# EthanD11/RS-VIO

Measured on AMD Instinct MI355X. Metric: stereo frames/sec (tracker+BA) on 752×480 EuRoC stream; BA ms/iter at window=10, higher is better.
Workload: dtype f32 (tracker) / f64 (BA)

## Files before the change

rs-vio_amd/csrc/pyramid.hip:

```cpp
#include "pyramid.hpp"

namespace rsvio {

namespace {

constexpr int TW = 64;
constexpr int TH = 8;
constexpr int STRIP_COLS = 320;
constexpr size_t LDS_CAP = 64 << 10;

__device__ __forceinline__ float triangle_kernel(float x) {
    float ax = fabsf(x);
    return ax < 1.0f ? 1.0f - ax : 0.0f;
}

__global__ void make_taps_kernel(TapTable tab, int n_entries) {
    int e = blockIdx.x * blockDim.x + threadIdx.x;
    if (e >= n_entries) return;
    int in_len = tab.ent_in_len[e];
    int out_len = tab.ent_out_len[e];
    int o = tab.ent_out_idx[e];
    float ratio = (float)in_len / (float)out_len;
    float sratio = ratio < 1.0f ? 1.0f : ratio;
    float support = 1.0f * sratio;
    float inputc = ((float)o + 0.5f) * ratio;
    long long left = (long long)floorf(inputc - support);
    if (left < 0) left = 0;
    if (left > (long long)in_len - 1) left = in_len - 1;
    long long right = (long long)ceilf(inputc + support);
    if (right < left + 1) right = left + 1;
    if (right > (long long)in_len) right = in_len;
    inputc = inputc - 0.5f;
    int cnt = (int)(right - left);
    float* w = tab.weights + (size_t)e * tab.max_taps;
    float sum = 0.0f;
    for (int k = 0; k < cnt; ++k) {
        float wv = triangle_kernel(((float)(left + k) - inputc) / sratio);
        w[k] = wv;
        sum += wv;
    }
    for (int k = 0; k < cnt; ++k) w[k] = w[k] / sum;
    tab.left[e] = (int)left;
    tab.count[e] = cnt;
}

__global__ __launch_bounds__(256) void pyramid_kernel(PyrLaunch L, PyrIO io) {
    extern __shared__ uint32_t smem[];
    const int img = blockIdx.y;
    {
        const int fb = (int)blockIdx.x - (L.copy_blocks + L.tile_start[L.levels]);
        if (fb >= 0) {
            if (io.table != nullptr) {
                const PyrSlot d = io.table[img];
                if (d.fast_pt != nullptr && fb < io.fast_cells)
                    fast_cell(d.src, io.fg, fb, nullptr, nullptr, 0, d.fast_pt, d.fast_aff,
                              reinterpret_cast<uint8_t*>(smem));
            } else if (img == 0 && fb < io.fast_cells) {
                const uint8_t* s0 = io.psrc ? io.psrc : io.src[0];
                fast_cell(s0, io.fg, fb, nullptr, nullptr, 0, io.fast_pt, io.fast_aff,
                          reinterpret_cast<uint8_t*>(smem));
            }
            return;
        }
    }
    const uint8_t* __restrict__ src =
        io.table ? io.table[img].src : (io.psrc ? io.psrc + (size_t)img * L.w * L.h : io.src[img]);
    uint8_t* __restrict__ dst_base =
        io.table ? io.table[img].dst : (io.psrc ? io.pdst + (size_t)img * L.pyr_bytes : io.dst[img]);
    int b = blockIdx.x;
    const bool aligned = ((reinterpret_cast<uintptr_t>(src) | reinterpret_cast<uintptr_t>(dst_base)) & 15) == 0;
    if (b < L.copy_blocks) {
        const size_t tot = (size_t)L.w * L.h;
        if (!aligned) {
            for (size_t i = (size_t)b * blockDim.x + threadIdx.x; i < tot; i += (size_t)L.copy_blocks * blockDim.x)
                dst_base[i] = src[i];
            return;
        }
        const size_t n16 = tot / 16;
        const uint4* s4 = reinterpret_cast<const uint4*>(src);
        uint4* d4 = reinterpret_cast<uint4*>(dst_base);
        for (size_t i = (size_t)b * blockDim.x + threadIdx.x; i < n16; i += (size_t)L.copy_blocks * blockDim.x)
            d4[i] = s4[i];
        size_t tail0 = n16 * 16;
        if (b == 0)
            for (size_t i = tail0 + threadIdx.x; i < tot; i += blockDim.x) dst_base[i] = src[i];
        return;
    }
    b -= L.copy_blocks;
    int lev = 1;
    while (lev < L.levels - 1 && b >= L.tile_start[lev + 1]) ++lev;
    b -= L.tile_start[lev];
    const int nw = (int)level_w(L.w, lev), nh = (int)level_h(L.h, lev);
    const int tw = L.tile_w[lev], th = L.tile_h[lev];
    const int tiles_x = (nw + tw - 1) / tw;
    const int tx = b % tiles_x, ty = b / tiles_x;
    const int ox0 = tx * tw, ox1 = min(ox0 + tw, nw);
    const int oy0 = ty * th, oy1 = min(oy0 + th, nh);
    const int rows = oy1 - oy0, cols_out = ox1 - ox0;
    const int hx = L.hx_ent[lev], vy = L.vy_ent[lev];
    const TapTable& T = L.tab;
    const int xl = T.left[hx + ox0];
    const int xr = T.left[hx + ox1 - 1] + T.count[hx + ox1 - 1];
    const int yl = T.left[vy + oy0];
    const int yr = T.left[vy + oy1 - 1] + T.count[vy + oy1 - 1];
    const int ncols = xr - xl, nrows = yr - yl;
    const int xa = xl & ~3, xoff = xl - xa;
    const int pd = (xr - xa + 3) >> 2;
    const bool direct = (L.direct >> lev) & 1;
    uint8_t* strip = reinterpret_cast<uint8_t*>(smem);
    if (!direct) {
        if (aligned && (L.w & 3) == 0) {
            const uint32_t* s32 = reinterpret_cast<const uint32_t*>(src);
            const int wd = (int)(L.w >> 2);
            for (int idx = threadIdx.x; idx < nrows * pd; idx += blockDim.x) {
                const int r = idx / pd, d = idx - r * pd;
                smem[idx] = s32[(size_t)(yl + r) * wd + (xa >> 2) + d];
            }
        } else {
            for (int idx = threadIdx.x; idx < nrows * pd * 4; idx += blockDim.x) {
                const int r = idx / (pd * 4), c = idx - r * pd * 4;
                strip[idx] = (xa + c < (int)L.w) ? src[(size_t)(yl + r) * L.w + xa + c] : 0;
            }
        }
    }
    float* tmp = reinterpret_cast<float*>(smem + (direct ? 0 : nrows * pd));
    __syncthreads();
    for (int idx = threadIdx.x; idx < rows * ncols; idx += blockDim.x) {
        const int r = idx / ncols, c = idx - r * ncols;
        const int e = vy + oy0 + r;
        const int vl = T.left[e], vc = T.count[e];
        const float* __restrict__ vw = T.weights + (size_t)e * T.max_taps;
        float acc = 0.0f;
        if (!direct) {
            const uint8_t* col = strip + (vl - yl) * pd * 4 + xoff + c;
            for (int k = 0; k < vc; ++k) acc += (float)col[k * pd * 4] * vw[k];
        } else {
            const uint8_t* __restrict__ col = src + (size_t)vl * L.w + xl + c;
            for (int k = 0; k < vc; k += 8) {
                float px[8];
#pragma unroll
                for (int u = 0; u < 8; ++u) px[u] = (k + u < vc) ? (float)col[(size_t)(k + u) * L.w] : 0.0f;
#pragma unroll
                for (int u = 0; u < 8; ++u)
                    if (k + u < vc) acc += px[u] * vw[k + u];
            }
        }
        tmp[r * ncols + c] = acc;
    }
    __syncthreads();
    uint8_t* __restrict__ dst = dst_base + level_offset(L.w, L.h, lev);
    for (int idx = threadIdx.x; idx < rows * cols_out; idx += blockDim.x) {
        const int r = idx / cols_out, c = idx - r * cols_out;
        const int e = hx + ox0 + c;
        const int hl = T.left[e] - xl, hc = T.count[e];
        const float* __restrict__ hw = T.weights + (size_t)e * T.max_taps;
        const float* __restrict__ row = tmp + r * ncols + hl;
        float acc = 0.0f;
        for (int k = 0; k < hc; ++k) acc += row[k] * hw[k];
        float cl = acc < 0.0f ? 0.0f : (acc > 255.0f ? 255.0f : acc);
        dst[(size_t)(oy0 + r) * nw + ox0 + c] = (uint8_t)roundf(cl);
    }
}

}

void PyramidPlan::init(int w_, int h_, int levels_) {
    w = w_;
    h = h_;
    levels = levels_;
    if (levels < 1 || levels > kMaxLevels) throw std::invalid_argument("levels must be in [1, 8]");
    if (w < 16 || h < 16) throw std::invalid_argument("image too small");
    std::vector<int> in_len, out_len, out_idx;
    float max_ratio = 1.0f;
    memset(&launch, 0, sizeof(launch));
    for (int i = 1; i < levels; ++i) {
        int nw = (int)level_w(w, i), nh = (int)level_h(h, i);
        if (nw < 1 || nh < 1) throw std::invalid_argument("too many levels for image size");
        launch.hx_ent[i] = (int)in_len.size();
        for (int o = 0; o < nw; ++o) { in_len.push_back(w); out_len.push_back(nw); out_idx.push_back(o); }
        launch.vy_ent[i] = (int)in_len.size();
        for (int o = 0; o < nh; ++o) { in_len.push_back(h); out_len.push_back(nh); out_idx.push_back(o); }
        float rx = (float)w / nw, ry = (float)h / nh;
        max_ratio = std::max(max_ratio, std::max(rx, ry));
        launch.tile_h[i] = std::max(1, std::min(TH, (int)(16.0f / ry)));
        launch.tile_w[i] = std::max(1, std::min(TW, (int)std::floor((STRIP_COLS - 2.0f * rx - 4.0f) / rx)));
    }
    n_entries = (int)in_len.size();
    max_taps = (int)std::ceil(2.0f * max_ratio) + 4;
    int tiles = 0;
    for (int i = 1; i < levels; ++i) {
        launch.tile_start[i] = tiles;
        int nw = (int)level_w(w, i), nh = (int)level_h(h, i);
        tiles += ((nw + launch.tile_w[i] - 1) / launch.tile_w[i]) * ((nh + launch.tile_h[i] - 1) / launch.tile_h[i]);
    }
    launch.tile_start[levels] = tiles;
    launch.copy_blocks = std::max(1, (int)(((size_t)w * h / 16 + 255) / 256 / 4));
    total_blocks = launch.copy_blocks + tiles;
    launch.w = (uint32_t)w;
    launch.h = (uint32_t)h;
    launch.levels = levels;
    launch.pyr_bytes = level_offset(w, h, levels);
    if (n_entries > 0) {
        i_in.alloc(n_entries); i_out.alloc(n_entries); i_idx.alloc(n_entries);
        d_left.alloc(n_entries); d_count.alloc(n_entries);
        d_w.alloc((size_t)n_entries * max_taps);
        RSVIO_HIP(hipMemcpy(i_in.p, in_len.data(), sizeof(int) * n_entries, hipMemcpyHostToDevice));
        RSVIO_HIP(hipMemcpy(i_out.p, out_len.data(), sizeof(int) * n_entries, hipMemcpyHostToDevice));
        RSVIO_HIP(hipMemcpy(i_idx.p, out_idx.data(), sizeof(int) * n_entries, hipMemcpyHostToDevice));
        TapTable t;
        t.left = d_left.p; t.count = d_count.p; t.weights = d_w.p; t.max_taps = max_taps;
        t.ent_in_len = i_in.p; t.ent_out_len = i_out.p; t.ent_out_idx = i_idx.p;
        hipLaunchKernelGGL(make_taps_kernel, dim3((n_entries + 255) / 256), dim3(256), 0, 0, t, n_entries);
        RSVIO_HIP(hipGetLastError());
        RSVIO_HIP(hipDeviceSynchronize());
        launch.tab = t;
        std::vector<int> left(n_entries), count(n_entries);
        RSVIO_HIP(hipMemcpy(left.data(), d_left.p, sizeof(int) * n_entries, hipMemcpyDeviceToHost));
        RSVIO_HIP(hipMemcpy(count.data(), d_count.p, sizeof(int) * n_entries, hipMemcpyDeviceToHost));
        for (int i = 1; i < levels; ++i) {
            const int nw = (int)level_w(w, i), nh = (int)level_h(h, i);
            const int tw = launch.tile_w[i], th = launch.tile_h[i];
            size_t strip = 0, vert = 0;
            for (int ox0 = 0; ox0 < nw; ox0 += tw) {
                const int ox1 = std::min(ox0 + tw, nw);
                const int xl = left[launch.hx_ent[i] + ox0];
                const int xr = left[launch.hx_ent[i] + ox1 - 1] + count[launch.hx_ent[i] + ox1 - 1];
                const size_t pd = (size_t)(xr - (xl & ~3) + 3) / 4;
                for (int oy0 = 0; oy0 < nh; oy0 += th) {
                    const int oy1 = std::min(oy0 + th, nh);
                    const int yl = left[launch.vy_ent[i] + oy0];
                    const int yr = left[launch.vy_ent[i] + oy1 - 1] + count[launch.vy_ent[i] + oy1 - 1];
                    strip = std::max(strip, 4 * pd * (size_t)(yr - yl));
                    vert = std::max(vert, 4 * (size_t)(oy1 - oy0) * (size_t)(xr - xl));
                }
            }
            if (vert > LDS_CAP) throw std::invalid_argument("image too wide for the pyramid tile");
            if (strip + vert > LDS_CAP) launch.direct |= 1u << i;
            lds_bytes = std::max(lds_bytes, ((launch.direct >> i) & 1) ? vert : strip + vert);
        }
    }
}

void PyramidPlan::enqueue(const PyrIO& io, int n_img, hipStream_t s) const {
    if (n_img <= 0) return;
    if (n_img > (io.psrc || io.table ? 65535 : kMaxPyrIO)) throw std::invalid_argument("too many images per pyramid launch");
    const size_t lds = io.fast_cells > 0 ? std::max(lds_bytes, (size_t)io.fg.g * io.fg.g) : lds_bytes;
    hipLaunchKernelGGL(pyramid_kernel, dim3(total_blocks + std::max(io.fast_cells, 0), n_img), dim3(256), lds, s,
                       launch, io);
    RSVIO_HIP(hipGetLastError());
}

void PyramidPlan::enqueue(const uint8_t* d_imgs, int n_img, uint8_t* d_pyrs, hipStream_t s) const {
    for (int i0 = 0; i0 < n_img; i0 += 65535) {
        PyrIO io{};
        io.psrc = d_imgs + (size_t)i0 * w * h;
        io.pdst = d_pyrs + (size_t)i0 * pyr_bytes();
        enqueue(io, std::min(65535, n_img - i0), s);
    }
}

}
```

rs-vio_amd/csrc/pyramid.hpp:

```cpp
#pragma once
#include <algorithm>
#include <cmath>
#include <cstring>
#include <stdexcept>
#include <vector>

#include "common.hpp"
#include "fast.hpp"

namespace rsvio {

constexpr int kMaxLevels = 8;

struct TapTable {
    int* left = nullptr;
    int* count = nullptr;
    float* weights = nullptr;
    int max_taps = 0;
    const int* ent_in_len = nullptr;
    const int* ent_out_len = nullptr;
    const int* ent_out_idx = nullptr;
};

struct PyrLaunch {
    uint32_t w, h;
    int levels;
    size_t pyr_bytes;
    int copy_blocks;
    int tile_start[kMaxLevels + 1];
    int tile_w[kMaxLevels];
    int tile_h[kMaxLevels];
    uint32_t direct;
    int hx_ent[kMaxLevels];
    int vy_ent[kMaxLevels];
    TapTable tab;
};

constexpr int kMaxPyrIO = 8;
struct PyrSlot {
    const uint8_t* src;
    uint8_t* dst;
    int4* fast_pt;
    float* fast_aff;
};
struct PyrIO {
    const uint8_t* src[kMaxPyrIO];
    uint8_t* dst[kMaxPyrIO];
    const uint8_t* psrc;
    uint8_t* pdst;
    int fast_cells;
    GridGeom fg;
    int4* fast_pt;
    float* fast_aff;
    const PyrSlot* table;
};

struct PyramidPlan {
    int w = 0, h = 0, levels = 0;
    int n_entries = 0, max_taps = 0, total_blocks = 0;
    size_t lds_bytes = 0;
    PyrLaunch launch;
    DevBuf<int> i_in, i_out, i_idx, d_left, d_count;
    DevBuf<float> d_w;
    void init(int w, int h, int levels);
    size_t pyr_bytes() const { return level_offset(w, h, levels); }
    void enqueue(const uint8_t* d_imgs, int n_img, uint8_t* d_pyrs, hipStream_t s) const;
    void enqueue(const PyrIO& io, int n_img, hipStream_t s) const;
};

}
```

rs-vio_amd/csrc/tracker.hip:

```cpp
#include <cmath>
#include <cstring>
#include <mutex>
#include <stdexcept>
#include <string>
#include <vector>

#include "lk_track.hpp"
#include "pyramid.hpp"
#include "camera.hpp"
#include "fast.hpp"

namespace rsvio {

namespace {

thread_local std::string g_last_error;

__device__ int block_exclusive_scan(int v, int* sh, int* total) {
    const int tid = threadIdx.x, lane = tid & 63, wave = tid >> 6, nw = blockDim.x >> 6;
    int incl = v;
#pragma unroll
    for (int off = 1; off < 64; off <<= 1) {
        const int t = __shfl_up(incl, off, 64);
        if (lane >= off) incl += t;
// ... 1060 lines not shown
            float* out[2] = {seeds_l, seeds_r};
            const size_t cp[2] = {cap_l, cap_r};
            std::vector<uint8_t> f;
            for (int k = 0; k < 2; ++k) {
                const size_t n = (size_t)T.pred_n[slot][k];
                f.assign(n, 0);
                if (n) RSVIO_HIP(hipMemcpy(f.data(), T.pflag(slot, k), n, hipMemcpyDeviceToHost));
                for (size_t i = 0; i < n; ++i) (f[i] ? c.n_seeded : c.n_unseeded)[k] += 1;
                if (!out[k]) continue;
                const size_t m = std::min(n, cp[k]);
                if (m) RSVIO_HIP(hipMemcpy(out[k], T.pseed(slot, k), m * sizeof(float2), hipMemcpyDeviceToHost));
                truncated = truncated || m < n;
            }
        }
        if (counts) *counts = c;
        if (truncated) {
            rsvio::set_last_error("rsvio_tracker_prediction_report: more seeds than the output capacity (truncated)");
            return (int)RSVIO_ERR_CAPACITY;
        }
        return (int)RSVIO_OK;
    });
}

int rsvio_tracker_remove_ids(rsvio_tracker* t, const uint64_t* ids, size_t n) {
    if (!t || (!ids && n)) return RSVIO_ERR_INVALID_ARG;
    if (n == 0) return RSVIO_OK;
    return guarded([&] {
        auto& T = t->t;
        T.require_collected("rsvio_tracker_remove_ids");
        if (T.rm_ids.n < n) T.rm_ids.alloc(n);
        RSVIO_HIP(hipMemcpyAsync(T.rm_ids.p, ids, n * sizeof(uint64_t), hipMemcpyHostToDevice, T.stream));
        hipLaunchKernelGGL(rsvio::remove_ids_kernel, dim3(1), dim3(1024), 0, T.stream, T.rm_ids.p, (int)n, T.maff(0),
                           T.maff(1), T.mid(0), T.mid(1), T.tmp_aff.p, T.ids_tmp.p, T.counts.p, T.outp(T.rslot, 0),
                           T.outp(T.rslot, 1), T.undp(T.rslot, 0), T.undp(T.rslot, 1), T.tmp_und.p);
        RSVIO_HIP(hipGetLastError());
        RSVIO_HIP(hipMemcpyAsync(T.h_counts.p, T.counts.p, sizeof(int) * 2, hipMemcpyDeviceToHost, T.stream));
        RSVIO_HIP(hipStreamSynchronize(T.stream));
        T.host_count[0] = T.h_counts.p[0];
        T.host_count[1] = T.h_counts.p[1];
        T.coll_n[0] = std::min(T.host_count[0], T.cap);
        T.coll_n[1] = std::min(T.host_count[1], T.cap);
        if (T.cams.on) {
            const size_t nl = std::min(T.last_n[0], (size_t)T.host_count[0]);
            const size_t nr = std::min(T.last_n[1], (size_t)T.host_count[1]);
            if (nl) RSVIO_HIP(hipMemcpyAsync(T.hund(T.rslot, 0), T.undp(T.rslot, 0), nl * sizeof(float2), hipMemcpyDeviceToHost, T.stream));
            if (nr) RSVIO_HIP(hipMemcpyAsync(T.hund(T.rslot, 1), T.undp(T.rslot, 1), nr * sizeof(float2),
                                             hipMemcpyDeviceToHost, T.stream));
            RSVIO_HIP(hipStreamSynchronize(T.stream));
            T.last_n[0] = nl;
            T.last_n[1] = nr;
        }
        return (int)RSVIO_OK;
    });
}

size_t rsvio_pyramid_bytes(int32_t w, int32_t h, int32_t levels) {
    if (w <= 0 || h <= 0 || levels <= 0) return 0;
    return rsvio::level_offset((uint32_t)w, (uint32_t)h, levels);
}

int rsvio_track_ctx_create(int32_t w, int32_t h, int32_t levels, int32_t device, rsvio_track_ctx** out) {
    if (!out) return RSVIO_ERR_INVALID_ARG;
    return guarded([&] {
        RSVIO_HIP(hipSetDevice(device));
        auto* c = new rsvio_track_ctx();
        try {
            c->c.device = device;
            c->c.plan.init(w, h, levels);
        } catch (...) {
            delete c;
            throw;
        }
        *out = c;
        return (int)RSVIO_OK;
    });
}

void rsvio_track_ctx_destroy(rsvio_track_ctx* c) { delete c; }

int rsvio_build_pyramids_d(rsvio_track_ctx* c, const uint8_t* d_imgs, int32_t n_img, uint8_t* d_pyrs, void* stream) {
    if (!c || !d_imgs || !d_pyrs || n_img < 0) return RSVIO_ERR_INVALID_ARG;
    return guarded([&] {
        c->c.plan.enqueue(d_imgs, n_img, d_pyrs, (hipStream_t)stream);
        return (int)RSVIO_OK;
    });
}

int rsvio_track_points_d(rsvio_track_ctx* c, const rsvio_track_batch* batches, int32_t n_batches,
                         int32_t max_iterations, float thresh, void* stream) {
    if (!c || !batches || n_batches < 0 || n_batches > rsvio::kMaxTrackBatches) return RSVIO_ERR_INVALID_ARG;
    return guarded([&] {
        rsvio::TrackLaunch L{};
        L.w = c->c.plan.w; L.h = c->c.plan.h; L.levels = c->c.plan.levels;
        L.max_iter = max_iterations; L.thresh = thresh; L.nb = n_batches;
        L.start[0] = 0;
        for (int b = 0; b < n_batches; ++b) {
            if (batches[b].n < 0) throw std::invalid_argument("negative batch size");
            L.start[b + 1] = L.start[b] + batches[b].n;
            L.pyr0[b] = batches[b].d_pyr0; L.pyr1[b] = batches[b].d_pyr1;
            L.ain[b] = batches[b].d_aff_in; L.aout[b] = batches[b].d_aff_out; L.valid[b] = batches[b].d_valid;
            L.dcount[b] = nullptr;
        }
        rsvio::enqueue_track(L, (hipStream_t)stream);
        return (int)RSVIO_OK;
    });
}

int rsvio_track_points_table_d(rsvio_track_ctx* c, const rsvio_track_batch* d_table, const int32_t* d_start,
                               int32_t n_batches, int32_t total, int32_t max_iterations, float thresh,
                               void* stream) {
    if (!c || n_batches < 0 || total < 0 || (n_batches > 0 && (!d_table || !d_start))) return RSVIO_ERR_INVALID_ARG;
    if (n_batches == 0 || total == 0) return RSVIO_OK;
    return guarded([&] {
        rsvio::TrackLaunch L{};
        L.w = c->c.plan.w; L.h = c->c.plan.h; L.levels = c->c.plan.levels;
        L.max_iter = max_iterations; L.thresh = thresh; L.nb = n_batches;
        L.start[0] = total;
        L.table = d_table;
        L.tstart = d_start;
        rsvio::enqueue_track(L, (hipStream_t)stream);
        return (int)RSVIO_OK;
    });
}

int rsvio_build_pyramid(const uint8_t* img, int32_t w, int32_t h, int32_t levels, uint8_t* out) {
    if (!img || !out) return RSVIO_ERR_INVALID_ARG;
    return guarded([&] {
        rsvio::PyramidPlan plan;
        plan.init(w, h, levels);
        rsvio::DevBuf<uint8_t> di((size_t)w * h), dp(plan.pyr_bytes());
        RSVIO_HIP(hipMemcpy(di.p, img, (size_t)w * h, hipMemcpyHostToDevice));
        plan.enqueue(di.p, 1, dp.p, nullptr);
        RSVIO_HIP(hipMemcpy(out, dp.p, plan.pyr_bytes(), hipMemcpyDeviceToHost));
        return (int)RSVIO_OK;
    });
}

int rsvio_dbg_pyramid_plan(int32_t w, int32_t h, int32_t levels, int32_t* tile_w, int32_t* tile_h, uint32_t* direct,
                           uint64_t* lds_bytes) {
    if (!tile_w || !tile_h || !direct || !lds_bytes) return RSVIO_ERR_INVALID_ARG;
    return guarded([&] {
        rsvio::PyramidPlan plan;
        plan.init(w, h, levels);
        for (int i = 0; i < rsvio::kMaxLevels; ++i) {
            tile_w[i] = plan.launch.tile_w[i];
            tile_h[i] = plan.launch.tile_h[i];
        }
        *direct = plan.launch.direct;
        *lds_bytes = (uint64_t)plan.lds_bytes;
        return (int)RSVIO_OK;
    });
}

int rsvio_track_points(const uint8_t* pyr0, const uint8_t* pyr1, int32_t w, int32_t h, int32_t levels,
                       const float* aff_in, int32_t n, int32_t max_iterations, float thresh, float* aff_out,
                       uint8_t* valid_out) {
    if (!pyr0 || !pyr1 || n < 0 || (n > 0 && (!aff_in || !aff_out || !valid_out))) return RSVIO_ERR_INVALID_ARG;
    if (levels < 1 || levels > rsvio::kMaxLevels || w < 1 || h < 1) return RSVIO_ERR_INVALID_ARG;
    return guarded([&] {
        const size_t pb = rsvio::level_offset(w, h, levels);
        rsvio::DevBuf<uint8_t> d0(pb), d1(pb), dv(std::max(n, 1));
        rsvio::DevBuf<float> ai((size_t)std::max(n, 1) * 6), ao((size_t)std::max(n, 1) * 6);
        RSVIO_HIP(hipMemcpy(d0.p, pyr0, pb, hipMemcpyHostToDevice));
        RSVIO_HIP(hipMemcpy(d1.p, pyr1, pb, hipMemcpyHostToDevice));
        if (n) RSVIO_HIP(hipMemcpy(ai.p, aff_in, sizeof(float) * 6 * n, hipMemcpyHostToDevice));
        rsvio::TrackLaunch L{};
        L.w = w; L.h = h; L.levels = levels; L.max_iter = max_iterations; L.thresh = thresh; L.nb = 1;
        L.start[0] = 0; L.start[1] = n;
        L.pyr0[0] = d0.p; L.pyr1[0] = d1.p; L.ain[0] = ai.p; L.aout[0] = ao.p; L.valid[0] = dv.p;
        L.dcount[0] = nullptr;
        rsvio::enqueue_track(L, nullptr);
        if (n) {
            RSVIO_HIP(hipMemcpy(aff_out, ao.p, sizeof(float) * 6 * n, hipMemcpyDeviceToHost));
            RSVIO_HIP(hipMemcpy(valid_out, dv.p, n, hipMemcpyDeviceToHost));
        }
        return (int)RSVIO_OK;
    });
}

int rsvio_track_points_seeded(const uint8_t* pyr0, const uint8_t* pyr1, int32_t w, int32_t h, int32_t levels,
                              const float* aff_in, const float* seeds, int32_t n, int32_t max_iterations, float thresh,
                              float* aff_out, uint8_t* valid_out) {
    if (!pyr0 || !pyr1 || n < 0 || (n > 0 && (!aff_in || !seeds || !aff_out || !valid_out))) return RSVIO_ERR_INVALID_ARG;
    if (levels < 1 || levels > rsvio::kMaxLevels || w < 1 || h < 1) return RSVIO_ERR_INVALID_ARG;
    return guarded([&] {
        const size_t pb = rsvio::level_offset(w, h, levels);
        const size_t m = (size_t)std::max(n, 1);
        rsvio::DevBuf<uint8_t> d0(pb), d1(pb), dv(m);
        rsvio::DevBuf<float> ai(m * 6), ao(m * 6), sd(m * 2);
        RSVIO_HIP(hipMemcpy(d0.p, pyr0, pb, hipMemcpyHostToDevice));
        RSVIO_HIP(hipMemcpy(d1.p, pyr1, pb, hipMemcpyHostToDevice));
        if (n) {
            RSVIO_HIP(hipMemcpy(ai.p, aff_in, sizeof(float) * 6 * n, hipMemcpyHostToDevice));
            RSVIO_HIP(hipMemcpy(sd.p, seeds, sizeof(float) * 2 * n, hipMemcpyHostToDevice));
        }
        rsvio::TrackLaunch L{};
        L.w = w; L.h = h; L.levels = levels; L.max_iter = max_iterations; L.thresh = thresh; L.nb = 1;
        L.start[0] = 0; L.start[1] = n;
        L.pyr0[0] = d0.p; L.pyr1[0] = d1.p; L.ain[0] = ai.p; L.aout[0] = ao.p; L.valid[0] = dv.p;
        L.dcount[0] = nullptr;
        rsvio::TrackSeeds S{};
        S.seed[0] = sd.p;
        rsvio::enqueue_track_seeded(L, S, nullptr);
        if (n) {
            RSVIO_HIP(hipMemcpy(aff_out, ao.p, sizeof(float) * 6 * n, hipMemcpyDeviceToHost));
            RSVIO_HIP(hipMemcpy(valid_out, dv.p, n, hipMemcpyDeviceToHost));
        }
        return (int)RSVIO_OK;
    });
}

int rsvio_detect_keypoints(const uint8_t* img, int32_t w, int32_t h, int32_t grid, const float* existing_xy,
                           int32_t n_existing, uint32_t* out_xy, float* out_score, int32_t cap, int32_t* n_out) {
    if (!img || !out_xy || !n_out || n_existing < 0 || (n_existing && !existing_xy) || grid < 8 || grid > 128 ||
        grid > w || grid > h)
        return RSVIO_ERR_INVALID_ARG;
    return guarded([&] {
        rsvio::GridGeom G = rsvio::make_grid(w, h, grid);
        const int n_cells = G.cells_x * G.cells_y;
        const int ne = std::max(n_existing, 1);
        rsvio::DevBuf<uint8_t> di((size_t)w * h);
        rsvio::DevBuf<float> ea((size_t)ne * 6), na((size_t)n_cells * 6), ns(n_cells);
        rsvio::DevBuf<int> nc(1);
        rsvio::DevBuf<int4> cp(n_cells);
        RSVIO_HIP(hipMemcpy(di.p, img, (size_t)w * h, hipMemcpyHostToDevice));
        std::vector<float> aff((size_t)ne * 6, 0.0f);
        for (int i = 0; i < n_existing; ++i) {
            aff[6 * i + 4] = existing_xy[2 * i];
            aff[6 * i + 5] = existing_xy[2 * i + 1];
        }
        RSVIO_HIP(hipMemcpy(ea.p, aff.data(), sizeof(float) * aff.size(), hipMemcpyHostToDevice));
        hipLaunchKernelGGL(rsvio::fast_cells_kernel, dim3(n_cells), dim3(256), (size_t)grid * grid, nullptr, di.p, G,
                           ea.p, nullptr, n_existing, cp.p, nullptr);
        RSVIO_HIP(hipGetLastError());
        hipLaunchKernelGGL(rsvio::gather_new_kernel, dim3(1), dim3(1024), 0, nullptr, cp.p, n_cells, na.p, nc.p, ns.p);
        RSVIO_HIP(hipGetLastError());
        int m = 0;
        RSVIO_HIP(hipMemcpy(&m, nc.p, sizeof(int), hipMemcpyDeviceToHost));
        std::vector<float> a((size_t)std::max(m, 1) * 6), sc(std::max(m, 1));
        if (m) {
            RSVIO_HIP(hipMemcpy(a.data(), na.p, sizeof(float) * 6 * m, hipMemcpyDeviceToHost));
            RSVIO_HIP(hipMemcpy(sc.data(), ns.p, sizeof(float) * m, hipMemcpyDeviceToHost));
        }
        const int k = std::min(m, cap);
        for (int i = 0; i < k; ++i) {
            out_xy[2 * i] = (uint32_t)a[6 * i + 4];
            out_xy[2 * i + 1] = (uint32_t)a[6 * i + 5];
            if (out_score) out_score[i] = sc[i];
        }
        *n_out = k;
        return m > cap ? (int)RSVIO_ERR_CAPACITY : (int)RSVIO_OK;
    });
}

}
```

rs-vio_amd/rsvio/_lib.py:

```python
from __future__ import annotations

import ctypes as C
import os
from pathlib import Path

PKG_ROOT = Path(__file__).resolve().parent.parent
LIB_PATH = PKG_ROOT / "lib" / "librsvio_gpu.so"

RSVIO_OK = 0
ERRORS = {
    -1: "RSVIO_ERR_INVALID_ARG", -2: "RSVIO_ERR_HIP", -3: "RSVIO_ERR_NOMEM", -4: "RSVIO_ERR_CAPACITY",
    -5: "RSVIO_ERR_NO_DEVICE", -6: "RSVIO_ERR_INTERNAL", -7: "RSVIO_ERR_RCCL",
}
LM_STATUS = {1: "CostToleranceReached", 2: "ParameterToleranceReached", 3: "MaxIterationsReached",
             4: "TrustRegionRadiusTooSmall", -1: "NumericalFailure", -2: "Skipped", -3: "LinearSolveFailed"}


class RsvioError(RuntimeError):
    def __init__(self, code: int, msg: str):
        super().__init__(f"{ERRORS.get(code, code)}: {msg}")
        self.code = code


class TrackerParams(C.Structure):
# ... 67 lines not shown
                ("reserved", C.c_int32), ("cost", C.c_double), ("min_pivot", C.c_double), ("kernel_ms", C.c_double)]


MCOV_STATUS = {1: "Ok", -1: "TooFew", -2: "Singular"}


class StereoFrame(C.Structure):
    _fields_ = [("left", C.c_void_p), ("right", C.c_void_p), ("stride", C.c_size_t),
                ("out_l", C.c_void_p), ("cap_l", C.c_size_t), ("out_r", C.c_void_p), ("cap_r", C.c_size_t),
                ("n_l", C.c_size_t), ("n_r", C.c_size_t), ("on_device", C.c_int32), ("status", C.c_int32)]


class StereoGate(C.Structure):
    _fields_ = [("mode", C.c_int32), ("reserved", C.c_int32), ("max_error", C.c_double),
                ("T_Cl_Cr", C.c_double * 16)]


class GateCounts(C.Structure):
    _fields_ = [("n_pairs", C.c_int32), ("n_rejected", C.c_int32), ("n_invalid", C.c_int32),
                ("reserved", C.c_int32)]


GATE_MODES = {"off": 0, "drop_right": 1, "drop_both": 2}


class TrackPrediction(C.Structure):
    _fields_ = [("R_l", C.c_double * 9), ("R_r", C.c_double * 9)]


class PredictionCounts(C.Structure):
    _fields_ = [("n_seeded", C.c_int32 * 2), ("n_unseeded", C.c_int32 * 2)]


class BaParams(C.Structure):
    _fields_ = [("max_keyframes", C.c_int32), ("max_landmarks", C.c_int32),
                ("max_observations", C.c_int32), ("device", C.c_int32)]


class LandmarkGate(C.Structure):
    _fields_ = [("mode", C.c_int32), ("reserved", C.c_int32), ("min_depth", C.c_double),
                ("max_depth", C.c_double), ("max_sq_error", C.c_double)]


class LandmarkInfo(C.Structure):
    _fields_ = [("n_obs", C.c_int32), ("flags", C.c_int32), ("min_depth", C.c_double),
                ("max_depth", C.c_double), ("max_sq_error", C.c_double)]


class CovInfo(C.Structure):
    _fields_ = [("status", C.c_int32), ("n_free", C.c_int32), ("n_singular", C.c_int32), ("reserved", C.c_int32),
                ("cost", C.c_double), ("device_ms", C.c_double)]


class BaLandmarkSlot(C.Structure):
    _fields_ = [("lm_mask", C.c_void_p), ("gate", C.POINTER(LandmarkGate)), ("p_W_out", C.c_void_p),
                ("info_out", C.c_void_p), ("n_lm", C.c_int32), ("n_ok", C.c_int32), ("status", C.c_int32),
                ("reserved", C.c_int32)]


class BaCovSlot(C.Structure):
    _fields_ = [("cov_cc", C.c_void_p), ("cov_pose", C.c_void_p), ("lm_idx", C.c_void_p), ("cov_lm", C.c_void_p),
                ("lm_flags", C.c_void_p), ("n_sel", C.c_int32), ("reserved", C.c_int32), ("info", CovInfo)]


LANDMARK_INFO_DTYPE = [("n_obs", "<i4"), ("flags", "<i4"), ("min_depth", "<f8"), ("max_depth", "<f8"),
                       ("max_sq_error", "<f8")]


class FtConfig(C.Structure):
    _fields_ = [("width", C.c_int32), ("height", C.c_int32), ("nlevels", C.c_int32),
                ("preprocessing_blur", C.c_int32), ("ratio", C.c_double), ("preprocessing_blur_sigma", C.c_float),
                ("detection_threshold", C.c_float), ("detection_min_dist", C.c_uint32), ("detection_blur", C.c_float),
                ("optical_flow_max_iter", C.c_int32), ("optical_flow_lm_lambda", C.c_float),
                ("matching_cost", C.c_int32), ("device", C.c_int32), ("max_features", C.c_int32),
                ("reserved", C.c_int32)]


class FtFeature(C.Structure):
    _fields_ = [("feature_id", C.c_uint64), ("x", C.c_float), ("y", C.c_float)]


P = C.c_void_p
SIG = {
    "rsvio_last_error": (C.c_char_p, []),
    "rsvio_device_info": (C.c_int, [C.c_int, C.c_char_p, C.c_size_t, C.POINTER(C.c_int)]),
    "rsvio_tracker_create": (C.c_int, [C.POINTER(TrackerParams), C.POINTER(P)]),
    "rsvio_tracker_destroy": (None, [P]),
    "rsvio_tracker_process_frame": (C.c_int, [P, P, P, C.c_size_t, P, C.c_size_t, C.POINTER(C.c_size_t), P,
                                              C.c_size_t, C.POINTER(C.c_size_t)]),
    "rsvio_tracker_process_frame_device": (C.c_int, [P, P, P, P, C.c_size_t, C.POINTER(C.c_size_t), P,
                                                     C.c_size_t, C.POINTER(C.c_size_t)]),
    "rsvio_window_problem": (C.c_int, [C.c_int32, P, P, P, P, P, P, P, C.c_int32, P, P, P, C.c_int32, P, P,
                                       C.POINTER(C.c_int32), C.c_int32, P, P, P, P, C.POINTER(C.c_int32)]),
    "rsvio_window_apply": (C.c_int, [C.c_int32, P, C.c_int32, P, P, P, P, P]),
    "rsvio_tracker_submit": (C.c_int, [P, P, P, C.c_size_t]),
    "rsvio_tracker_submit_device": (C.c_int, [P, P, P]),
    "rsvio_tracker_collect": (C.c_int, [P, P, C.c_size_t, C.POINTER(C.c_size_t), P, C.c_size_t,
                                        C.POINTER(C.c_size_t)]),
    "rsvio_tracker_remove_ids": (C.c_int, [P, P, C.c_size_t]),
    "rsvio_tracker_stream": (P, [P]),
    "rsvio_sincosf": (C.c_int, [P, C.c_size_t, P, P]),
    "rsvio_sincosf_digest": (C.c_int, [C.c_uint64, C.c_uint64, C.c_uint32, P]),
    "rsvio_unproject": (C.c_int, [C.POINTER(Camera), P, C.c_size_t, P, P]),
    "rsvio_unproject_d": (C.c_int, [C.POINTER(Camera), P, C.c_size_t, P, P, P]),
    "rsvio_tracker_set_cameras": (C.c_int, [P, C.POINTER(Camera), C.POINTER(Camera)]),
    "rsvio_tracker_undistorted": (C.c_int, [P, P, C.c_size_t, P, C.c_size_t]),
    "rsvio_quat_from_matrix": (C.c_int, [P, C.c_size_t, P]),
    "rsvio_pnp_create": (C.c_int, [C.c_int32, C.POINTER(P)]),
    "rsvio_pnp_destroy": (None, [P]),
    "rsvio_pnp_set_stream": (C.c_int, [P, P]),
    "rsvio_pnp_set_map": (C.c_int, [P, P, P, C.c_int32]),
    "rsvio_track_motion": (C.c_int, [P, P, P, C.c_size_t, P, P, C.c_size_t, P, P, C.POINTER(LmCfg),
                                     C.POINTER(KeyframeRule), C.POINTER(MotionResult)]),
    "rsvio_track_motion_tracker": (C.c_int, [P, P, P, P, C.POINTER(LmCfg), C.POINTER(KeyframeRule),
                                             C.POINTER(MotionResult)]),
    "rsvio_track_motion_robust": (C.c_int, [P, P, P, C.c_size_t, P, P, C.c_size_t, P, P, C.POINTER(LmCfg),
                                            C.POINTER(KeyframeRule), C.POINTER(RansacCfg), P, P, P, P,
                                            C.POINTER(RobustMotionResult)]),
    "rsvio_track_motion_robust_tracker": (C.c_int, [P, P, P, P, C.POINTER(LmCfg), C.POINTER(KeyframeRule),
                                                    C.POINTER(RansacCfg), P, P, P, P,
                                                    C.POINTER(RobustMotionResult)]),
    "rsvio_pnp_batch_create": (C.c_int, [P, C.c_int32, C.POINTER(P)]),
    "rsvio_pnp_batch_track_motion": (C.c_int, [P, P, C.POINTER(LmCfg), C.POINTER(KeyframeRule), P,
                                               C.POINTER(C.c_double)]),
    "rsvio_pnp_batch_track_motion_robust": (C.c_int, [P, P, C.POINTER(LmCfg), C.POINTER(KeyframeRule),
                                                      C.POINTER(RansacCfg), P, C.POINTER(C.c_double)]),
    "rsvio_pnp_batch_destroy": (None, [P]),
    "rsvio_motion_covariance": (C.c_int, [P, P, P, C.c_size_t, P, P, C.c_size_t, P, P, P, P, C.c_double, P,
                                          C.POINTER(MotionCovInfo)]),
    "rsvio_motion_covariance_tracker": (C.c_int, [P, P, P, P, P, P, C.c_double, P, C.POINTER(MotionCovInfo)]),
    "rsvio_pnp_batch_covariance": (C.c_int, [P, P, P, C.c_double, P, P, C.POINTER(C.c_double)]),
    "rsvio_tracker_batch_create": (C.c_int, [P, C.c_int32, C.POINTER(P)]),
    "rsvio_tracker_batch_process_frames": (C.c_int, [P, P, C.POINTER(C.c_double)]),
    "rsvio_tracker_batch_destroy": (None, [P]),
    "rsvio_tracker_device_lists": (C.c_int, [P, C.POINTER(P), C.POINTER(C.c_size_t), C.POINTER(P),
                                             C.POINTER(C.c_size_t), C.POINTER(P), C.POINTER(P)]),
    "rsvio_tracker_set_stereo_gate": (C.c_int, [P, C.POINTER(StereoGate)]),
    "rsvio_tracker_gate_report": (C.c_int, [P, C.POINTER(GateCounts), P, P, C.c_size_t, C.POINTER(C.c_size_t)]),
    "rsvio_stereo_gate_lists": (C.c_int, [C.POINTER(StereoGate), C.c_int32, C.c_int32, P, P, C.c_size_t, P, P,
                                          C.c_size_t, P, P, P, C.POINTER(GateCounts)]),
    "rsvio_project": (C.c_int, [C.POINTER(Camera), P, C.c_size_t, P, P]),
    "rsvio_project_d": (C.c_int, [C.POINTER(Camera), P, C.c_size_t, P, P, P]),
    "rsvio_predict_seeds": (C.c_int, [C.POINTER(Camera), P, P, C.c_size_t, C.c_int32, C.c_int32, P, P]),
    "rsvio_predict_seeds_d": (C.c_int, [C.POINTER(Camera), P, P, C.c_size_t, C.c_int32, C.c_int32, P, P, P]),
    "rsvio_track_points_seeded": (C.c_int, [P, P, C.c_int32, C.c_int32, C.c_int32, P, P, C.c_int32, C.c_int32,
                                            C.c_float, P, P]),
    "rsvio_tracker_set_prediction": (C.c_int, [P, C.POINTER(TrackPrediction)]),
    "rsvio_tracker_prediction_report": (C.c_int, [P, C.POINTER(PredictionCounts), P, C.c_size_t, P, C.c_size_t]),
    "rsvio_dbg_stereo_gate_frame": (C.c_int, [C.POINTER(StereoGate), C.c_int32, C.c_int32, P, P, P,
                                              C.POINTER(C.c_size_t), P, P, P, C.POINTER(C.c_size_t), P, P,
                                              C.POINTER(GateCounts)]),
    "rsvio_dbg_pyramid_plan": (C.c_int, [C.c_int32, C.c_int32, C.c_int32, P, P, C.POINTER(C.c_uint32),
                                         C.POINTER(C.c_uint64)]),
    "rsvio_pyramid_bytes": (C.c_size_t, [C.c_int32, C.c_int32, C.c_int32]),
    "rsvio_build_pyramid": (C.c_int, [P, C.c_int32, C.c_int32, C.c_int32, P]),
    "rsvio_track_points": (C.c_int, [P, P, C.c_int32, C.c_int32, C.c_int32, P, C.c_int32, C.c_int32, C.c_float,
                                     P, P]),
    "rsvio_detect_keypoints": (C.c_int, [P, C.c_int32, C.c_int32, C.c_int32, P, C.c_int32, P, P, C.c_int32,
                                         C.POINTER(C.c_int32)]),
    "rsvio_track_ctx_create": (C.c_int, [C.c_int32, C.c_int32, C.c_int32, C.c_int32, C.POINTER(P)]),
    "rsvio_track_ctx_destroy": (None, [P]),
    "rsvio_build_pyramids_d": (C.c_int, [P, P, C.c_int32, P, P]),
    "rsvio_track_points_d": (C.c_int, [P, C.POINTER(TrackBatch), C.c_int32, C.c_int32, C.c_float, P]),
    "rsvio_track_points_table_d": (C.c_int, [P, P, P, C.c_int32, C.c_int32, C.c_int32, C.c_float, P]),
    "rsvio_ba_create": (C.c_int, [C.POINTER(BaParams), C.POINTER(P)]),
    "rsvio_ba_destroy": (None, [P]),
    "rsvio_ba_solve": (C.c_int, [P, C.c_int32, P, P, C.c_int32, P, C.c_int32, P, P, P, P, P,
                                 C.POINTER(LmCfg), C.POINTER(BaResult)]),
    "rsvio_ba_set_problem": (C.c_int, [P, C.c_int32, P, P, C.c_int32, P, C.c_int32, P, P, P, P, P]),
    "rsvio_ba_run": (C.c_int, [P, C.POINTER(LmCfg), C.POINTER(BaResult)]),
    "rsvio_ba_run_async": (C.c_int, [P, C.POINTER(LmCfg)]),
    "rsvio_ba_set_stream": (C.c_int, [P, P]),
    "rsvio_ba_batch_create": (C.c_int, [P, C.c_int32, C.POINTER(P)]),
    "rsvio_ba_batch_run": (C.c_int, [P, C.POINTER(LmCfg), P]),
    "rsvio_ba_batch_destroy": (None, [P]),
    "rsvio_ba_batch_run_active": (C.c_int, [P, P, C.POINTER(LmCfg), P]),
    "rsvio_ba_batch_triangulate": (C.c_int, [P, P, C.POINTER(LandmarkGate), P, C.POINTER(C.c_double)]),
    "rsvio_ba_batch_check_landmarks": (C.c_int, [P, P, C.POINTER(LandmarkGate), P, C.POINTER(C.c_double)]),
    "rsvio_ba_batch_covariance": (C.c_int, [P, P, C.c_double, P, C.POINTER(C.c_double)]),
    "rsvio_ba_p2p_export": (C.c_int, [P, C.c_int32, C.POINTER(C.c_uint8), C.c_size_t]),
    "rsvio_ba_attach_p2p": (C.c_int, [P, C.c_int32, C.c_int32, C.POINTER(C.c_uint8)]),
    "rsvio_ba_p2p_latency": (C.c_int, [P, C.c_int32, C.c_int32, C.POINTER(C.c_double)]),
    "rsvio_ba_detach_p2p": (C.c_int, [P]),
    "rsvio_ba_p2p_level": (C.c_int, [P, C.POINTER(C.c_int32)]),
    "rsvio_stream_create": (C.c_int, [C.c_int32, C.POINTER(C.c_uint32), C.c_uint32, C.POINTER(P)]),
    "rsvio_stream_destroy": (C.c_int, [P]),
    "rsvio_upload_async": (C.c_int, [P, P, C.c_size_t, P]),
    "rsvio_ba_wait": (C.c_int, [P, C.POINTER(BaResult)]),
    "rsvio_ba_get_state": (C.c_int, [P, P, P]),
    "rsvio_ba_triangulate": (C.c_int, [P, P, C.c_int32, C.POINTER(LandmarkGate), P, P, C.POINTER(C.c_int32)]),
    "rsvio_ba_check_landmarks": (C.c_int, [P, C.c_int32, C.POINTER(LandmarkGate), P, C.POINTER(C.c_int32)]),
    "rsvio_ba_covariance": (C.c_int, [P, C.c_double, P, P, P, C.c_int32, P, P, C.POINTER(CovInfo)]),
    "rsvio_ba_build_system": (C.c_int, [P, C.c_double, C.c_double, P, P, C.POINTER(C.c_double)]),
    "rsvio_rccl_unique_id": (C.c_int, [P, C.c_size_t]),
    "rsvio_ba_attach_comm": (C.c_int, [P, C.c_int32, C.c_int32, P]),
    "rsvio_ft_create": (C.c_int, [C.POINTER(FtConfig), C.POINTER(P)]),
    "rsvio_ft_destroy": (None, [P]),
    "rsvio_ft_process_frame": (C.c_int, [P, P, C.c_size_t, P, C.c_size_t, C.POINTER(C.c_size_t)]),
    "rsvio_ft_process_frame_device": (C.c_int, [P, P, P, C.c_size_t, C.POINTER(C.c_size_t)]),
    "rsvio_ft_get_pyramid": (C.c_int, [P, P, C.c_size_t]),
    "rsvio_ft_stream": (P, [P]),
    "rsvio_ft_pyramid_floats": (C.c_size_t, [C.c_int32, C.c_int32, C.c_int32, C.c_double]),
    "rsvio_ft_build_pyramid": (C.c_int, [P, C.c_int32, C.c_int32, C.c_int32, C.c_double, C.c_int32, C.c_float, P]),
    "rsvio_ft_track_points": (C.c_int, [P, P, C.c_int32, C.c_int32, C.c_int32, C.c_double, P, C.c_int32, C.c_int32,
                                        C.c_float, C.c_int32, P, P]),
    "rsvio_ft_shi_tomasi_score": (C.c_int, [P, C.c_int32, C.c_int32, C.c_float, P]),
    "rsvio_ft_add_points": (C.c_int, [P, C.c_int32, C.c_int32, P, C.c_int32, C.c_float, C.c_int32, C.c_float, P,
                                      C.c_int32, C.POINTER(C.c_int32)]),
}

_lib = None


def load() -> C.CDLL:
    global _lib
    if _lib is not None:
        return _lib
    path = Path(os.environ.get("RSVIO_LIB", LIB_PATH))
    if not path.exists():
        raise RuntimeError(f"{path} not found: build it with `make -C rs-vio_amd` (hipcc, gfx950); "
                           "rsvio has no CPU fallback")
    try:
        import torch
    except ImportError:
        pass
    lib = C.CDLL(str(path))
    for name, (res, args) in SIG.items():
        try:
            fn = getattr(lib, name)
        except AttributeError:
            continue
        fn.restype = res
        fn.argtypes = args
    _lib = lib
    return lib


def check(code: int) -> int:
    if code < 0:
        msg = load().rsvio_last_error()
        raise RsvioError(code, msg.decode() if msg else "")
    return code


def ptr(a) -> int | None:
    if a is None:
        return None
    ai = a.__array_interface__
    if ai["strides"] is not None and not a.flags["C_CONTIGUOUS"]:
        raise ValueError("array must be C-contiguous")
    return ai["data"][0]


def require_device(device: int = 0) -> str:
    lib = load()
    name = C.create_string_buffer(64)
    ncu = C.c_int(0)
    check(lib.rsvio_device_info(device, name, 64, C.byref(ncu)))
    return name.value.decode()


class CuStream:

    def __init__(self, device: int, cus=None):
        lib = load()
        out = C.c_void_p()
        if cus is None:
            check(lib.rsvio_stream_create(device, None, 0, C.byref(out)))
        else:
            n = max(cus) + 1
            words = (n + 31) // 32
            mask = (C.c_uint32 * words)()
            for c in cus:
                mask[c // 32] |= 1 << (c % 32)
            check(lib.rsvio_stream_create(device, mask, words, C.byref(out)))
        self.ptr = out.value

    def close(self):
        if self.ptr:
            check(load().rsvio_stream_destroy(self.ptr))
            self.ptr = None
```

Baseline: 5189.

## Stage tap tables in LDS and vectorize vertical pass in pyramid kernel

```diff
diff --git a/rs-vio_amd/csrc/pyramid.hip b/rs-vio_amd/csrc/pyramid.hip
--- a/rs-vio_amd/csrc/pyramid.hip
+++ b/rs-vio_amd/csrc/pyramid.hip
@@ -14,23 +14,27 @@
     return ax < 1.0f ? 1.0f - ax : 0.0f;
 }
 
+__device__ __forceinline__ void tap_span(int in_len, int out_len, int o, long long& left, long long& right,
+                                         float& inputc, float& sratio) {
+    float ratio = (float)in_len / (float)out_len;
+    sratio = ratio < 1.0f ? 1.0f : ratio;
+    float support = 1.0f * sratio;
+    inputc = ((float)o + 0.5f) * ratio;
+    left = (long long)floorf(inputc - support);
+    if (left < 0) left = 0;
+    if (left > (long long)in_len - 1) left = in_len - 1;
+    right = (long long)ceilf(inputc + support);
+    if (right < left + 1) right = left + 1;
+    if (right > (long long)in_len) right = in_len;
+    inputc = inputc - 0.5f;
+}
+
 __global__ void make_taps_kernel(TapTable tab, int n_entries) {
     int e = blockIdx.x * blockDim.x + threadIdx.x;
     if (e >= n_entries) return;
-    int in_len = tab.ent_in_len[e];
-    int out_len = tab.ent_out_len[e];
-    int o = tab.ent_out_idx[e];
-    float ratio = (float)in_len / (float)out_len;
-    float sratio = ratio < 1.0f ? 1.0f : ratio;
-    float support = 1.0f * sratio;
-    float inputc = ((float)o + 0.5f) * ratio;
-    long long left = (long long)floorf(inputc - support);
-    if (left < 0) left = 0;
-    if (left > (long long)in_len - 1) left = in_len - 1;
-    long long right = (long long)ceilf(inputc + support);
-    if (right < left + 1) right = left + 1;
-    if (right > (long long)in_len) right = in_len;
-    inputc = inputc - 0.5f;
+    long long left, right;
+    float inputc, sratio;
+    tap_span(tab.ent_in_len[e], tab.ent_out_len[e], tab.ent_out_idx[e], left, right, inputc, sratio);
     int cnt = (int)(right - left);
     float* w = tab.weights + (size_t)e * tab.max_taps;
     float sum = 0.0f;
@@ -42,6 +46,13 @@
     for (int k = 0; k < cnt; ++k) w[k] = w[k] / sum;
     tab.left[e] = (int)left;
     tab.count[e] = cnt;
+}
+
+__device__ __forceinline__ int div_tile(int n, int d, float rd) {
+    int q = (int)((float)n * rd);
+    const int rem = n - q * d;
+    q += (rem >= d) - (rem < 0);
+    return q;
 }
 
 __global__ __launch_bounds__(256) void pyramid_kernel(PyrLaunch L, PyrIO io) {
@@ -99,14 +110,132 @@
     const int rows = oy1 - oy0, cols_out = ox1 - ox0;
     const int hx = L.hx_ent[lev], vy = L.vy_ent[lev];
     const TapTable& T = L.tab;
-    const int xl = T.left[hx + ox0];
-    const int xr = T.left[hx + ox1 - 1] + T.count[hx + ox1 - 1];
-    const int yl = T.left[vy + oy0];
-    const int yr = T.left[vy + oy1 - 1] + T.count[vy + oy1 - 1];
+    int xl, xr, yl, yr;
+    {
+        long long l0, r0, l1, r1;
+        float c, s;
+        tap_span((int)L.w, nw, ox0, l0, r0, c, s);
+        tap_span((int)L.w, nw, ox1 - 1, l1, r1, c, s);
+        xl = (int)l0;
+        xr = (int)r1;
+        tap_span((int)L.h, nh, oy0, l0, r0, c, s);
+        tap_span((int)L.h, nh, oy1 - 1, l1, r1, c, s);
+        yl = (int)l0;
+        yr = (int)r1;
+    }
     const int ncols = xr - xl, nrows = yr - yl;
     const int xa = xl & ~3, xoff = xl - xa;
     const int pd = (xr - xa + 3) >> 2;
     const bool direct = (L.direct >> lev) & 1;
+    uint8_t* __restrict__ dst = dst_base + level_offset(L.w, L.h, lev);
+    if ((L.ltap >> lev) & 1) {
+        const int tid = threadIdx.x;
+        const int ne = rows + cols_out, tn = L.tap_n[lev];
+        const int nd = nrows * pd, nwt = ne * tn;
+        float* tmp = reinterpret_cast<float*>(smem + nd);
+        int* tl = reinterpret_cast<int*>(tmp + rows * ncols);
+        int* tc = tl + ne;
+        float* tws = reinterpret_cast<float*>(tc + ne);
+        const float rpd = 1.0f / (float)pd, rtn = 1.0f / (float)tn, rco = 1.0f / (float)cols_out;
+        const bool dwords = aligned && (L.w & 3) == 0;
+        const uint32_t* s32 = reinterpret_cast<const uint32_t*>(src);
+        const int wd = (int)(L.w >> 2);
+        constexpr int SU = 8, WU = 4;
+        uint32_t sv[SU];
+        float wv[WU];
+        int el = 0, ec = 0;
+        if (dwords) {
+#pragma unroll
+            for (int u = 0; u < SU; ++u) {
+                const int idx = tid + u * 256;
+                sv[u] = 0;
+                if (idx < nd) {
+                    const int r = div_tile(idx, pd, rpd), d = idx - r * pd;
+                    sv[u] = s32[(size_t)(yl + r) * wd + (xa >> 2) + d];
+                }
+            }
+        }
+#pragma unroll
+        for (int u = 0; u < WU; ++u) {
+            const int idx = tid + u * 256;
+            wv[u] = 0.0f;
+            if (idx < nwt) {
+                const int en = div_tile(idx, tn, rtn), k = idx - en * tn;
+                const int e = en < rows ? vy + oy0 + en : hx + ox0 + en - rows;
+                wv[u] = T.weights[(size_t)e * T.max_taps + k];
+            }
+        }
+        if (tid < ne) {
+            const int e = tid < rows ? vy + oy0 + tid : hx + ox0 + tid - rows;
+            el = T.left[e];
+            ec = T.count[e];
+        }
+        if (dwords) {
+#pragma unroll
+            for (int u = 0; u < SU; ++u) {
+                const int idx = tid + u * 256;
+                if (idx < nd) smem[idx] = sv[u];
+            }
+            for (int idx = tid + SU * 256; idx < nd; idx += 256) {
+                const int r = div_tile(idx, pd, rpd), d = idx - r * pd;
+                smem[idx] = s32[(size_t)(yl + r) * wd + (xa >> 2) + d];
+            }
+        } else {
+            uint8_t* strip = reinterpret_cast<uint8_t*>(smem);
+            for (int idx = tid; idx < nd * 4; idx += 256) {
+                const int r = div_tile(idx >> 2, pd, rpd), c = idx - r * pd * 4;
+                strip[idx] = (xa + c < (int)L.w) ? src[(size_t)(yl + r) * L.w + xa + c] : 0;
+            }
+        }
+#pragma unroll
+        for (int u = 0; u < WU; ++u) {
+            const int idx = tid + u * 256;
+            if (idx < nwt) tws[idx] = wv[u];
+        }
+        for (int idx = tid + WU * 256; idx < nwt; idx += 256) {
+            const int en = div_tile(idx, tn, rtn), k = idx - en * tn;
+            const int e = en < rows ? vy + oy0 + en : hx + ox0 + en - rows;
+            tws[idx] = T.weights[(size_t)e * T.max_taps + k];
+        }
+        if (tid < ne) {
+            tl[tid] = el;
+            tc[tid] = ec;
+        }
+        __syncthreads();
+        for (int idx = tid; idx < rows * pd; idx += 256) {
+            const int r = div_tile(idx, pd, rpd), j = idx - r * pd;
+            const int vc = tc[r];
+            const float* vw = tws + r * tn;
+            const uint32_t* col = smem + (tl[r] - yl) * pd + j;
+            float a0 = 0.0f, a1 = 0.0f, a2 = 0.0f, a3 = 0.0f;
+            for (int k = 0; k < vc; ++k) {
+                const uint32_t px = col[k * pd];
+                const float wk = vw[k];
+                a0 += (float)(px & 0xffu) * wk;
+                a1 += (float)((px >> 8) & 0xffu) * wk;
+                a2 += (float)((px >> 16) & 0xffu) * wk;
+                a3 += (float)(px >> 24) * wk;
+            }
+            const int c = 4 * j - xoff;
+            float* t = tmp + r * ncols + c;
+            if (c >= 0 && c < ncols) t[0] = a0;
+            if (c + 1 >= 0 && c + 1 < ncols) t[1] = a1;
+            if (c + 2 >= 0 && c + 2 < ncols) t[2] = a2;
+            if (c + 3 < ncols) t[3] = a3;
+        }
+        __syncthreads();
+        for (int idx = tid; idx < rows * cols_out; idx += 256) {
+            const int r = div_tile(idx, cols_out, rco), c = idx - r * cols_out;
+            const int hc = tc[rows + c];
+            const float* hw = tws + (rows + c) * tn;
+            const float* row = tmp + r * ncols + (tl[rows + c] - xl);
+            float acc = 0.0f;
+            for (int k = 0; k < hc; ++k) acc += row[k] * hw[k];
+            float cl = acc < 0.0f ? 0.0f : (acc > 255.0f ? 255.0f : acc);
+            dst[(size_t)(oy0 + r) * nw + ox0 + c] = (uint8_t)roundf(cl);
+        }
+        return;
+    }
     uint8_t* strip = reinterpret_cast<uint8_t*>(smem);
     if (!direct) {
         if (aligned && (L.w & 3) == 0) {
@@ -148,7 +277,6 @@
         tmp[r * ncols + c] = acc;
     }
     __syncthreads();
-    uint8_t* __restrict__ dst = dst_base + level_offset(L.w, L.h, lev);
     for (int idx = threadIdx.x; idx < rows * cols_out; idx += blockDim.x) {
         const int r = idx / cols_out, c = idx - r * cols_out;
         const int e = hx + ox0 + c;
@@ -217,6 +345,7 @@
         std::vector<int> left(n_entries), count(n_entries);
         RSVIO_HIP(hipMemcpy(left.data(), d_left.p, sizeof(int) * n_entries, hipMemcpyDeviceToHost));
         RSVIO_HIP(hipMemcpy(count.data(), d_count.p, sizeof(int) * n_entries, hipMemcpyDeviceToHost));
+        size_t lds_launch = 0;
         for (int i = 1; i < levels; ++i) {
             const int nw = (int)level_w(w, i), nh = (int)level_h(h, i);
             const int tw = launch.tile_w[i], th = launch.tile_h[i];
@@ -237,14 +366,25 @@
             if (vert > LDS_CAP) throw std::invalid_argument("image too wide for the pyramid tile");
             if (strip + vert > LDS_CAP) launch.direct |= 1u << i;
             lds_bytes = std::max(lds_bytes, ((launch.direct >> i) & 1) ? vert : strip + vert);
-        }
+            int tn = 1;
+            for (int e = launch.hx_ent[i]; e < launch.vy_ent[i] + nh; ++e) tn = std::max(tn, count[e]);
+            const size_t taps = 4 * (size_t)(th + tw) * (size_t)(2 + tn);
+            launch.tap_n[i] = tn;
+            if (!((launch.direct >> i) & 1) && strip + vert + taps <= LDS_CAP) {
+                launch.ltap |= 1u << i;
+                lds_launch = std::max(lds_launch, strip + vert + taps);
+            }
+        }
+        lds_launch = std::max(lds_launch, lds_bytes);
+        tap_lds = lds_launch - lds_bytes;
     }
 }
 
 void PyramidPlan::enqueue(const PyrIO& io, int n_img, hipStream_t s) const {
     if (n_img <= 0) return;
     if (n_img > (io.psrc || io.table ? 65535 : kMaxPyrIO)) throw std::invalid_argument("too many images per pyramid launch");
-    const size_t lds = io.fast_cells > 0 ? std::max(lds_bytes, (size_t)io.fg.g * io.fg.g) : lds_bytes;
+    const size_t lds_pyr = lds_bytes + tap_lds;
+    const size_t lds = io.fast_cells > 0 ? std::max(lds_pyr, (size_t)io.fg.g * io.fg.g) : lds_pyr;
     hipLaunchKernelGGL(pyramid_kernel, dim3(total_blocks + std::max(io.fast_cells, 0), n_img), dim3(256), lds, s,
                        launch, io);
     RSVIO_HIP(hipGetLastError());
diff --git a/rs-vio_amd/csrc/pyramid.hpp b/rs-vio_amd/csrc/pyramid.hpp
--- a/rs-vio_amd/csrc/pyramid.hpp
+++ b/rs-vio_amd/csrc/pyramid.hpp
@@ -33,6 +33,8 @@
     uint32_t direct;
     int hx_ent[kMaxLevels];
     int vy_ent[kMaxLevels];
+    uint32_t ltap;
+    int tap_n[kMaxLevels];
     TapTable tab;
 };
 
@@ -59,6 +61,7 @@
     int w = 0, h = 0, levels = 0;
     int n_entries = 0, max_taps = 0, total_blocks = 0;
     size_t lds_bytes = 0;
+    size_t tap_lds = 0;
     PyrLaunch launch;
     DevBuf<int> i_in, i_out, i_idx, d_left, d_count;
     DevBuf<float> d_w;
diff --git a/rs-vio_amd/csrc/tracker.hip b/rs-vio_amd/csrc/tracker.hip
--- a/rs-vio_amd/csrc/tracker.hip
+++ b/rs-vio_amd/csrc/tracker.hip
@@ -1236,6 +1236,61 @@
     });
 }
 
+int rsvio_dbg_pyramid_taps(int32_t w, int32_t h, int32_t levels, uint32_t* ltap, int32_t* tap_n, uint64_t* tap_lds) {
+    if (!ltap || !tap_n || !tap_lds) return RSVIO_ERR_INVALID_ARG;
+    return guarded([&] {
+        rsvio::PyramidPlan plan;
+        plan.init(w, h, levels);
+        for (int i = 0; i < rsvio::kMaxLevels; ++i) tap_n[i] = plan.launch.tap_n[i];
+        *ltap = plan.launch.ltap;
+        *tap_lds = (uint64_t)plan.tap_lds;
+        return (int)RSVIO_OK;
+    });
+}
+
+int rsvio_dbg_pyramid_launch(const uint8_t* imgs, int32_t n, int32_t w, int32_t h, int32_t levels, int32_t table,
+                             int32_t grid, uint8_t* out_pyrs, int32_t* out_cells) {
+    if (!imgs || !out_pyrs || n < 1 || n > rsvio::kMaxPyrIO || grid < 0) return RSVIO_ERR_INVALID_ARG;
+    return guarded([&] {
+        rsvio::PyramidPlan plan;
+        plan.init(w, h, levels);
+        const size_t img = (size_t)w * h, pb = plan.pyr_bytes();
+        rsvio::GridGeom G{};
+        if (grid > 0) G = rsvio::make_grid(w, h, grid);
+        const int n_cells = grid > 0 ? G.cells_x * G.cells_y : 0;
+        const int n_fast = grid > 0 ? (table ? n : 1) : 0;
+        rsvio::DevBuf<uint8_t> di(n * img), dp(n * pb);
+        rsvio::DevBuf<int4> cp((size_t)std::max(n_fast * n_cells, 1));
+        rsvio::DevBuf<float> ca((size_t)std::max(n_fast * n_cells, 1) * 6);
+        rsvio::DevBuf<rsvio::PyrSlot> dt(n);
+        RSVIO_HIP(hipMemcpy(di.p, imgs, n * img, hipMemcpyHostToDevice));
+        RSVIO_HIP(hipMemset(cp.p, 0, sizeof(int4) * std::max(n_fast * n_cells, 1)));
+        rsvio::PyrIO io{};
+        io.fast_cells = n_cells;
+        io.fg = G;
+        if (table) {
+            std::vector<rsvio::PyrSlot> slots(n);
+            for (int i = 0; i < n; ++i)
+                slots[i] = rsvio::PyrSlot{di.p + i * img, dp.p + i * pb, grid > 0 ? cp.p + (size_t)i * n_cells : nullptr,
+                                          grid > 0 ? ca.p + (size_t)i * n_cells * 6 : nullptr};
+            RSVIO_HIP(hipMemcpy(dt.p, slots.data(), sizeof(rsvio::PyrSlot) * n, hipMemcpyHostToDevice));
+            io.table = dt.p;
+        } else {
+            for (int i = 0; i < n; ++i) {
+                io.src[i] = di.p + i * img;
+                io.dst[i] = dp.p + i * pb;
+            }
+            io.fast_pt = grid > 0 ? cp.p : nullptr;
+            io.fast_aff = grid > 0 ? ca.p : nullptr;
+        }
+        plan.enqueue(io, n, nullptr);
+        RSVIO_HIP(hipMemcpy(out_pyrs, dp.p, n * pb, hipMemcpyDeviceToHost));
+        if (out_cells && n_fast * n_cells > 0)
+            RSVIO_HIP(hipMemcpy(out_cells, cp.p, sizeof(int4) * n_fast * n_cells, hipMemcpyDeviceToHost));
+        return (int)RSVIO_OK;
+    });
+}
+
 int rsvio_track_points(const uint8_t* pyr0, const uint8_t* pyr1, int32_t w, int32_t h, int32_t levels,
                        const float* aff_in, int32_t n, int32_t max_iterations, float thresh, float* aff_out,
                        uint8_t* valid_out) {
diff --git a/rs-vio_amd/rsvio/_lib.py b/rs-vio_amd/rsvio/_lib.py
--- a/rs-vio_amd/rsvio/_lib.py
+++ b/rs-vio_amd/rsvio/_lib.py
@@ -243,6 +243,9 @@
                                               C.POINTER(GateCounts)]),
     "rsvio_dbg_pyramid_plan": (C.c_int, [C.c_int32, C.c_int32, C.c_int32, P, P, C.POINTER(C.c_uint32),
                                          C.POINTER(C.c_uint64)]),
+    "rsvio_dbg_pyramid_taps": (C.c_int, [C.c_int32, C.c_int32, C.c_int32, C.POINTER(C.c_uint32), P,
+                                         C.POINTER(C.c_uint64)]),
+    "rsvio_dbg_pyramid_launch": (C.c_int, [P, C.c_int32, C.c_int32, C.c_int32, C.c_int32, C.c_int32, C.c_int32, P, P]),
     "rsvio_pyramid_bytes": (C.c_size_t, [C.c_int32, C.c_int32, C.c_int32]),
     "rsvio_build_pyramid": (C.c_int, [P, C.c_int32, C.c_int32, C.c_int32, P]),
     "rsvio_track_points": (C.c_int, [P, P, C.c_int32, C.c_int32, C.c_int32, P, C.c_int32, C.c_int32, C.c_float,
```

Result: slower. 5091 (-1.9%).
